# r9y9/deepvoice3_pytorch

Hardware: AMD Instinct MI355X
Metric: mel-frames/sec/node (train step, deepvoice3_ljspeech) (higher is better)
Workload: dtype f16x3

## Files before the change

### deepvoice3_pytorch_amd/csrc/api.hip

```cpp
#include "common.h"
#include <atomic>
#include <mutex>
#include <vector>
#include <string.h>

static thread_local char g_err[512] = "";

void dv3_set_error(const char* fmt, ...) {
  va_list ap;
  va_start(ap, fmt);
  vsnprintf(g_err, sizeof(g_err), fmt, ap);
  va_end(ap);
}

int g_dv3_last_conv = 0, g_dv3_last_wgrad = 0;

__device__ uint32_t g_dv3_range_events;
uint32_t* dv3_range_ctr() {
  static uint32_t* ptr = nullptr;
  static std::once_flag once;
  std::call_once(once, [] {
    void* p = nullptr;
    if (hipGetSymbolAddress(&p, HIP_SYMBOL(g_dv3_range_events)) == hipSuccess) ptr = (uint32_t*)p;
  });
// ... 194 lines not shown

extern "C" int dv3_device_info(int dev, char* name, int name_len, int* n_cu) {
  hipDeviceProp_t prop;
  hipError_t e = hipGetDeviceProperties(&prop, dev);
  if (e != hipSuccess) {
    dv3_set_error("hipGetDeviceProperties: %s", hipGetErrorString(e));
    return DV3_ELAUNCH;
  }
  if (name && name_len > 0) {
    strncpy(name, prop.gcnArchName, (size_t)name_len - 1);
    name[name_len - 1] = 0;
  }
  if (n_cu) *n_cu = prop.multiProcessorCount;
  return DV3_OK;
}

extern "C" int dv3_sizeof(const char* name) {
#define DV3_SZ(T) if (!strcmp(name, #T)) return (int)sizeof(T)
  DV3_SZ(dv3_conv_desc);
  DV3_SZ(dv3_wgrad_desc);
  DV3_SZ(dv3_wn_desc);
  DV3_SZ(dv3_wn_bwd_desc);
  DV3_SZ(dv3_gate_bwd_desc);
  DV3_SZ(dv3_softmax_desc);
  DV3_SZ(dv3_softmax_bwd_desc);
  DV3_SZ(dv3_spec_loss_desc);
  DV3_SZ(dv3_spec_items_desc);
  DV3_SZ(dv3_wn_multi_entry);
  DV3_SZ(dv3_conv_step_desc);
  DV3_SZ(dv3_attn_step_desc);
  DV3_SZ(dv3_decode_entry);
  DV3_SZ(dv3_decode_program);
  DV3_SZ(dv3_attn_fwd_desc);
  DV3_SZ(dv3_spk_layer);
  DV3_SZ(dv3_spk_desc);
  DV3_SZ(dv3_dropout_site);
  DV3_SZ(dv3_dtw_desc);
#undef DV3_SZ
  return -1;
}
```

### deepvoice3_pytorch_amd/csrc/attention.hip

```cpp
#include "common.h"

namespace {

__global__ __launch_bounds__(256) void attn_softmax_kernel(const dv3_softmax_desc p) {
  const int lane = threadIdx.x & 63;
  const int64_t row = (int64_t)blockIdx.x * 4 + (threadIdx.x >> 6);
  if (row >= (int64_t)p.B * p.Tq) return;
  const int b = (int)(row / p.Tq);
  const int Tk = p.Tk;
  float* s = p.s + row * Tk;
  int lo = 0, hi = Tk;
  if (p.key_len) hi = min(hi, p.key_len[b]);
  if (p.last_attended) {
    const int la = p.last_attended[0];
    const int wlo = la - p.win_back, whi = la + p.win_ahead;
    if (wlo > 0) lo = max(lo, wlo);
    if (whi < Tk) hi = min(hi, whi);
  }
  float mx = -INFINITY;
  for (int n = lo + lane; n < hi; n += 64) mx = fmaxf(mx, s[n]);
  mx = dv3_wave_max(mx);
  float sum = 0.f;
  for (int n = lo + lane; n < hi; n += 64) sum += expf(s[n] - mx);
  sum = dv3_wave_sum(sum);
// ... 15 lines not shown
__global__ __launch_bounds__(256) void attn_softmax_bwd_kernel(const dv3_softmax_bwd_desc p) {
  const int lane = threadIdx.x & 63;
  const int64_t row = (int64_t)blockIdx.x * 4 + (threadIdx.x >> 6);
  if (row >= (int64_t)p.B * p.Tq) return;
  const int Tk = p.Tk;
  const float* pr = p.p + row * Tk;
  const float* dpd = p.dpd ? p.dpd + row * Tk : nullptr;
  const float* dpx = p.dp_direct ? p.dp_direct + row * Tk : nullptr;
  float* ds = p.ds + row * Tk;
  const float drop_scale = p.scale_dev ? p.drop_scale * p.scale_dev[0] : p.drop_scale;
  float dot = 0.f;
  for (int n = lane; n < Tk; n += 64) {
    float d = 0.f;
    if (dpd) {
      d = dpd[n] * drop_scale;
      if (p.mask && !dv3_keep(p.mask, row, p.mask_rs, n)) d = 0.f;
    }
    if (dpx) d += dpx[n];
    dot += d * pr[n];
  }
  dot = dv3_wave_sum(dot);
  for (int n = lane; n < Tk; n += 64) {
    float d = 0.f;
    if (dpd) {
      d = dpd[n] * drop_scale;
      if (p.mask && !dv3_keep(p.mask, row, p.mask_rs, n)) d = 0.f;
    }
    if (dpx) d += dpx[n];
    ds[n] = pr[n] * (d - dot);
  }
}

typedef float f32x2v __attribute__((ext_vector_type(2)));
__global__ __launch_bounds__(256) void attn_fwd_kernel(const dv3_attn_fwd_desc p) {
  extern __shared__ float sc[];
  const int tid = threadIdx.x, lane = tid & 63, wave = tid >> 6;
  const int l31 = lane & 31, lhi = lane >> 5;
  const int b = blockIdx.y, t0 = blockIdx.x * 32;
  const int E = p.E, Tq = p.Tq, Tk = p.Tk;
  const int ld = Tk + 1;
  const int nkt = (Tk + 31) / 32;
  const float* __restrict__ qb = p.q + (int64_t)b * E * Tq;
  const float* __restrict__ kb = p.k + (int64_t)b * E * Tk;
  const int tq = min(t0 + l31, Tq - 1);
  for (int kt = wave; kt < nkt; kt += 4) {
    const int n = min(kt * 32 + l31, Tk - 1);
    f32x16 acc;
#pragma unroll
    for (int r = 0; r < 16; ++r) acc[r] = 0.f;
    auto fetch1 = [&](int e0, float (&a)[16], float (&bv)[16]) __attribute__((always_inline)) {
#pragma unroll
      for (int i = 0; i < 16; ++i) {
        const int e = e0 + 2 * i + lhi;
        const int ee = min(e, E - 1);
        const float av = qb[(int64_t)ee * Tq + tq];
        bv[i] = kb[(int64_t)ee * Tk + n];
        a[i] = e < E ? av : 0.f;
      }
    };
    float a0[16], b0[16], a1[16], b1[16];
    fetch1(0, a0, b0);
    for (int e0 = 0; e0 < E; e0 += 64) {
      if (e0 + 32 < E) fetch1(e0 + 32, a1, b1);
#pragma unroll
      for (int i = 0; i < 16; ++i) acc = __builtin_amdgcn_mfma_f32_32x32x2f32(a0[i], b0[i], acc, 0, 0, 0);
      if (e0 + 32 >= E) break;
      if (e0 + 64 < E) fetch1(e0 + 64, a0, b0);
// ... 8 lines not shown
  }
  __syncthreads();
  {
    const int row = tid >> 3, sub = tid & 7;
    const int t = t0 + row;
    int hi = Tk;
    if (p.key_len) hi = min(hi, p.key_len[b]);
    float* s = sc + row * ld;
    float mx = -INFINITY;
    for (int n = sub; n < hi; n += 8) mx = fmaxf(mx, s[n]);
#pragma unroll
    for (int off = 4; off > 0; off >>= 1) mx = fmaxf(mx, __shfl_xor(mx, off, 64));
    float sum = 0.f;
    for (int n = sub; n < hi; n += 8) sum += expf(s[n] - mx);
#pragma unroll
    for (int off = 4; off > 0; off >>= 1) sum += __shfl_xor(sum, off, 64);
    const float inv = 1.0f / sum;
    const float pd_scale = p.pd_scale_dev ? p.pd_scale * p.pd_scale_dev[0] : p.pd_scale;
    const int64_t grow = (int64_t)b * Tq + t;
    for (int n = sub; n < Tk; n += 8) {
      float v = 0.f;
      if (n < hi) v = expf(s[n] - mx) * inv;
      float d = v;
      if (p.mask && t < Tq) d = dv3_keep(p.mask, grow, p.mask_rs, n) ? v * p.drop_scale : 0.f;
      d *= pd_scale;
      s[n] = d;
      if (t < Tq) {
        p.P[grow * Tk + n] = v;
        p.pd[grow * Tk + n] = d;
      }
    }
  }
  __syncthreads();
  const float* __restrict__ vtb = p.vT + (int64_t)b * Tk * E;
  for (int et = wave; et * 32 < E; et += 4) {
    const int e = min(et * 32 + l31, E - 1);
    f32x16 acc;
#pragma unroll
    for (int r = 0; r < 16; ++r) acc[r] = 0.f;
    auto fetch3 = [&](int n0, float (&a)[16], float (&bv)[16]) __attribute__((always_inline)) {
#pragma unroll
      for (int i = 0; i < 16; ++i) {
        const int n = n0 + 2 * i + lhi;
        const int nn = min(n, Tk - 1);
        const float av = vtb[(int64_t)nn * E + e];
        bv[i] = sc[l31 * ld + nn];
        a[i] = n < Tk ? av : 0.f;
      }
    };
    float a0[16], b0[16], a1[16], b1[16];
    fetch3(0, a0, b0);
    for (int n0 = 0; n0 < Tk; n0 += 64) {
      if (n0 + 32 < Tk) fetch3(n0 + 32, a1, b1);
#pragma unroll
      for (int i = 0; i < 16; ++i) acc = __builtin_amdgcn_mfma_f32_32x32x2f32(a0[i], b0[i], acc, 0, 0, 0);
      if (n0 + 32 >= Tk) break;
      if (n0 + 64 < Tk) fetch3(n0 + 64, a0, b0);
#pragma unroll
      for (int i = 0; i < 16; ++i) acc = __builtin_amdgcn_mfma_f32_32x32x2f32(a1[i], b1[i], acc, 0, 0, 0);
    }
    const int t = t0 + l31;
    if (t < Tq) {
#pragma unroll
      for (int r = 0; r < 16; ++r) {
        const int ec = et * 32 + (r & 3) + 8 * (r >> 2) + 4 * lhi;
        if (ec < E) p.ctx[((int64_t)b * E + ec) * Tq + t] = acc[r];
      }
    }
  }
}

__global__ __launch_bounds__(64) void attn_argmax_kernel(const float* __restrict__ p, int Tk,
                                                         int32_t* __restrict__ out) {
  const int lane = threadIdx.x;
  float best = -INFINITY;
  int bi = 0x7fffffff;
  for (int n = lane; n < Tk; n += 64) {
    const float v = p[n];
    if (v > best) { best = v; bi = n; }
  }
#pragma unroll
  for (int off = 32; off > 0; off >>= 1) {
    const float ov = __shfl_xor(best, off, 64);
    const int oi = __shfl_xor(bi, off, 64);
    if (ov > best || (ov == best && oi < bi)) { best = ov; bi = oi; }
  }
  if (lane == 0) out[0] = bi;
}

}

extern "C" int dv3_attn_softmax_f32(const dv3_softmax_desc* d, void* stream) {
  DV3_REQUIRE(d && d->s && d->B > 0 && d->Tq > 0 && d->Tk > 0, "attn_softmax: bad args");
  if (d->mask) DV3_REQUIRE(d->pd && d->mask_rs * 32 >= d->Tk, "attn_softmax: mask needs pd and a wide enough row stride");
  const int64_t rows = (int64_t)d->B * d->Tq;
  hipLaunchKernelGGL(attn_softmax_kernel, dim3((unsigned)dv3_cdiv64(rows, 4)), dim3(256), 0,
                     (hipStream_t)stream, *d);
  return dv3_check_launch("attn_softmax_f32");
}

extern "C" int dv3_attn_softmax_bwd_f32(const dv3_softmax_bwd_desc* d, void* stream) {
  DV3_REQUIRE(d && d->p && d->ds && (d->dpd || d->dp_direct), "attn_softmax_bwd: bad args");
  DV3_REQUIRE(d->B > 0 && d->Tq > 0 && d->Tk > 0, "attn_softmax_bwd: bad dims");
  const int64_t rows = (int64_t)d->B * d->Tq;
  hipLaunchKernelGGL(attn_softmax_bwd_kernel, dim3((unsigned)dv3_cdiv64(rows, 4)), dim3(256), 0,
                     (hipStream_t)stream, *d);
  return dv3_check_launch("attn_softmax_bwd_f32");
}

extern "C" int dv3_attn_fwd_f32(const dv3_attn_fwd_desc* d, void* stream) {
  DV3_REQUIRE(d && d->q && d->k && d->vT && d->ctx && d->P && d->pd, "attn_fwd: null pointer");
  DV3_REQUIRE(d->B > 0 && d->E > 0 && d->Tq > 0 && d->Tk > 0 && d->B <= 65535, "attn_fwd: bad dims");
  if (d->mask) DV3_REQUIRE(d->mask_rs * 32 >= d->Tk, "attn_fwd: mask row stride too small");
  const size_t lds = (size_t)32 * (d->Tk + 1) * sizeof(float);
  DV3_REQUIRE(lds <= 64 * 1024, "attn_fwd: Tk = %d too long for the fused kernel (use the unfused path)", d->Tk);
  hipLaunchKernelGGL(attn_fwd_kernel, dim3(dv3_cdiv(d->Tq, 32), d->B), dim3(256), lds, (hipStream_t)stream, *d);
  return dv3_check_launch("attn_fwd");
}

extern "C" int dv3_attn_argmax_i32(const float* p_row, int32_t Tk, int32_t* out, void* stream) {
  DV3_REQUIRE(p_row && out && Tk > 0, "attn_argmax: bad args");
  hipLaunchKernelGGL(attn_argmax_kernel, dim3(1), dim3(64), 0, (hipStream_t)stream, p_row, Tk, out);
  return dv3_check_launch("attn_argmax_i32");
}
```

### deepvoice3_pytorch_amd/ops.py

```python
import contextlib
import ctypes
import functools
import math

import torch

from . import _lib
from ._lib import CONSTS, STRUCTS, _env_flag, _env_int, _env_str

EPI_LINEAR = CONSTS["DV3_EPI_LINEAR"]
EPI_RELU = CONSTS["DV3_EPI_RELU"]
EPI_SIGMOID = CONSTS["DV3_EPI_SIGMOID"]
EPI_GLU = CONSTS["DV3_EPI_GLU"]
EPI_HIGHWAY = CONSTS["DV3_EPI_HIGHWAY"]
EPI_DGRAD = CONSTS["DV3_EPI_DGRAD"]
EPI_SOFTSIGN = CONSTS["DV3_EPI_SOFTSIGN"]
STORE_BCT = CONSTS["DV3_STORE_BCT"]
STORE_INTERLEAVE2 = CONSTS["DV3_STORE_INTERLEAVE2"]

_conv_desc = STRUCTS["dv3_conv_desc"]
_wgrad_desc = STRUCTS["dv3_wgrad_desc"]
_wn_desc = STRUCTS["dv3_wn_desc"]
_wn_bwd_desc = STRUCTS["dv3_wn_bwd_desc"]
_gate_bwd_desc = STRUCTS["dv3_gate_bwd_desc"]
_softmax_desc = STRUCTS["dv3_softmax_desc"]
_softmax_bwd_desc = STRUCTS["dv3_softmax_bwd_desc"]
_attn_fwd_desc = STRUCTS["dv3_attn_fwd_desc"]
_spec_loss_desc = STRUCTS["dv3_spec_loss_desc"]
_spec_items_desc = STRUCTS["dv3_spec_items_desc"]


_GEMM_MODES = ("f16x3", "bf16x3", "f32", "bf16")
_gemm_mode = _env_str("DV3_GEMM", "f16x3")
if _gemm_mode not in _GEMM_MODES:
    raise RuntimeError("DV3_GEMM must be one of %s" % (_GEMM_MODES,))


def set_gemm_precision(mode):
    global _gemm_mode
    if mode not in _GEMM_MODES:
        raise ValueError("gemm precision must be one of %s" % (_GEMM_MODES,))
    prev, _gemm_mode = _gemm_mode, mode
    return prev


def gemm_precision():
    return _gemm_mode


_raw_stream = getattr(torch._C, "_cuda_getCurrentRawStream", None)
_cur_device = getattr(torch._C, "_cuda_getDevice", None)
import threading as _threading


class _StreamOverride(_threading.local):
    handle = None


_stream_override = _StreamOverride()

# ... 289 lines not shown
            pk.fwd_s._dv3_f16 = f16
            e = tab[n]
            e.d.v, e.d.g, e.d.scale = v.data_ptr(), _ptr(g), pk.scale.data_ptr()
            e.d.lda, e.d.a_half, e.d.ldb = pk.lda, pk.a_half, pk.ldb
            e.d.O, e.d.I, e.d.J, e.d.transposed, e.d.glu_cg = O, I, J, 0, glu_cg
            e.d.fwd_dtype = SPLIT_F16 if f16 else SPLIT_BF16
            e.fwd_split, e.bwd_split = pk.fwd_s.data_ptr(), pk.bwd_s.data_ptr()
            first_row.append(rows)
            first_block.append(blocks)
            rows += O
            blocks += ((O + 31) // 32) * ((I + 31) // 32)
            max_j = max(max_j, J)
            self.by_id[id(v)] = (pk, v.data_ptr(), glu_cg)
        raw = torch.frombuffer(bytearray(bytes(tab)), dtype=torch.uint8)
        self.table = raw.to(dev)
        self.first_row = torch.tensor(first_row, dtype=torch.int32, device=dev)
        self.first_block = torch.tensor(first_block, dtype=torch.int32, device=dev)
        self.n, self.rows, self.blocks, self.max_j = len(layers), rows, blocks, max_j
        self.keep = layers

    def run(self):
        _lib.call("dv3_weight_norm_split_pack_multi", self.table.data_ptr(), self.first_row.data_ptr(),
                  self.first_block.data_ptr(), self.n, self.rows, self.blocks, self.max_j, _stream())

    def lookup(self, v, glu_cg):
        hit = self.by_id.get(id(v))
        if hit is None or hit[1] != v.data_ptr() or hit[2] != glu_cg or self.mode != _gemm_mode:
            return None
        return hit[0]


prepacked = None
fused_attention = _env_flag("DV3_FUSED_ATTN", True)


bf16_storage = _env_flag("DV3_BF16_STORAGE", True)


def zero_(t):
    _lib.call("dv3_memset_b8", t.data_ptr(), 0, t.numel() * t.element_size(), _stream())
    return t


def storage_c8():
    return bf16_storage and _gemm_mode == "bf16"


def c8_groups(C):
    return _round_up(C, 32) // 8


def is_c8(t):
    return t is not None and t.dim() == 4 and t.dtype == torch.bfloat16 and t.shape[-1] == 8


def _c8_empty(B, C, T, device):
    shape = (B, c8_groups(C), T, 8)
    t = torch.empty(shape, dtype=torch.bfloat16, device=device)
    if C % 32:
        G, g0 = c8_groups(C), C // 8
        _lib.call("dv3_memset_rows_b8", t.data_ptr() + g0 * T * 16, 0, B, (G - g0) * T * 16, G * T * 16, _stream())
    t._dv3_C = C
    return t


def _c8_C(t, C=None):
# ... 1207 lines not shown
    if (x8 or want8) and not _c8_layer_ok(v, cfg, x8 if want8 is None else bool(want8), x.shape[2]):
        y = ConvLayerFn.apply(from_c8(x, v.shape[1]) if x8 else x, v, g, bias, spk,
                              from_c8(r) if is_c8(r) else r, from_c8(r2) if is_c8(r2) else r2, cfg, packed)
        out8 = x8 if want8 is None else bool(want8)
        return to_c8(y) if out8 else y
    if x8 or want8:
        y = ConvLayerC8Fn.apply(x, v, g, bias, spk, r, r2, cfg, packed)
        if is_c8(y):
            gated = cfg.mode in (EPI_GLU, EPI_HIGHWAY)
            y._dv3_C = v.shape[0] // 2 if gated else v.shape[0]
        return y
    return ConvLayerFn.apply(x, v, g, bias, spk, r, r2, cfg, packed)


def _attn_split(forward=False):
    if forward and _gemm_mode == "f16x3":
        return False
    return _gemm_mode != "f32"


class AttnCoreFn(torch.autograd.Function):
    @staticmethod
    def forward(ctx, q, k, v, key_len, last_attended, cfg):
        q, k, v = _c(_chk(q, "q")), _c(_chk(k, "k")), _c(_chk(v, "v"))
        B, E, Tq = q.shape
        Tk = k.shape[2]
        p_drop, training, win_back, win_ahead, site = cfg
        dev = q.device
        bits, bits_rs, dscale = None, 0, 1.0
        if training and p_drop > 0:
            bits, bits_rs = dropout_bits(B * Tq, Tk, p_drop, dev, site)
            dscale = 1.0 / (1.0 - p_drop)
        if fused_attention and last_attended is None and Tk <= 511 and Tq > 1:
            vT = transpose(v)
            ctxv = torch.empty((B, E, Tq), dtype=torch.float32, device=dev)
            P = torch.empty((B, Tq, Tk), dtype=torch.float32, device=dev)
            pd = torch.empty_like(P)
            d = _attn_fwd_desc()
            d.q, d.k, d.vT, d.key_len = q.data_ptr(), k.data_ptr(), vT.data_ptr(), _ptr(key_len)
            d.mask, d.mask_rs, d.drop_scale = _ptr(bits), bits_rs, dscale
            vs = valid.scale if valid is not None else None
            d.pd_scale = 1.0 if vs is not None else Tk * math.sqrt(1.0 / Tk)
            d.pd_scale_dev = _ptr(vs)
            d.ctx, d.P, d.pd = ctxv.data_ptr(), P.data_ptr(), pd.data_ptr()
            d.B, d.E, d.Tq, d.Tk = B, E, Tq, Tk
            _lib.call("dv3_attn_fwd_f32", ctypes.byref(d), _stream())
            if any(ctx.needs_input_grad[:3]):
                ctx.save_for_backward(q, k, v, P, pd)
                ctx.bits, ctx.bits_rs, ctx.dscale, ctx.pd_scale = bits, bits_rs, dscale, d.pd_scale
                ctx.scale_dev = vs
            return ctxv, P
        S = conv_gemm(k, q, Tq, 0, B=B, Cin=E, Tin=Tk, M=Tq, Tout=Tk, a_bs=E * Tq)
        pd = torch.empty_like(S)
        d = _softmax_desc()
        d.s, d.pd, d.key_len, d.last_attended = S.data_ptr(), pd.data_ptr(), _ptr(key_len), _ptr(last_attended)
        d.mask, d.mask_rs, d.drop_scale = _ptr(bits), bits_rs, dscale
        vs = valid.scale if valid is not None else None
        d.pd_scale = 1.0 if vs is not None else Tk * math.sqrt(1.0 / Tk)
        d.pd_scale_dev = _ptr(vs)
        d.B, d.Tq, d.Tk, d.win_back, d.win_ahead = B, Tq, Tk, win_back, win_ahead
        _lib.call("dv3_attn_softmax_f32", ctypes.byref(d), _stream())
        P = S
        ctxv = wgrad_gemm(v, pd, B=B, M=E, Cin=Tq, T=Tk, Tin=Tk, n_slabs=B,
                          split_bf16=_attn_split(forward=True)).view(B, E, Tq)
        if any(ctx.needs_input_grad[:3]):
            ctx.save_for_backward(q, k, v, P, pd)
            ctx.bits, ctx.bits_rs, ctx.dscale, ctx.pd_scale = bits, bits_rs, dscale, d.pd_scale
            ctx.scale_dev = vs
        return ctxv, P

    @staticmethod
    def backward(ctx, dctx, dP):
        q, k, v, P, pd = ctx.saved_tensors
        B, E, Tq = q.shape
        Tk = k.shape[2]
        dctx = _c(dctx)
        pdT = transpose(pd)
        dv = wgrad_gemm(dctx, pdT, B=B, M=E, Cin=Tk, T=Tq, Tin=Tq, n_slabs=B, split_bf16=_attn_split()).view(B, E, Tk)
        dpd = conv_gemm(v, dctx, Tq, 0, B=B, Cin=E, Tin=Tk, M=Tq, Tout=Tk, a_bs=E * Tq)
        dS = torch.empty_like(P)
        d = _softmax_bwd_desc()
        d.p, d.dpd, d.ds = P.data_ptr(), dpd.data_ptr(), dS.data_ptr()
        d.dp_direct = _ptr(_c(dP)) if dP is not None else None
        d.mask, d.mask_rs, d.drop_scale = _ptr(ctx.bits), ctx.bits_rs, ctx.dscale * ctx.pd_scale
        d.scale_dev = _ptr(ctx.scale_dev)
        d.B, d.Tq, d.Tk = B, Tq, Tk
        _lib.call("dv3_attn_softmax_bwd_f32", ctypes.byref(d), _stream())
        dq = wgrad_gemm(k, dS, B=B, M=E, Cin=Tq, T=Tk, Tin=Tk, n_slabs=B, split_bf16=_attn_split()).view(B, E, Tq)
        dST = transpose(dS)
        dk = wgrad_gemm(q, dST, B=B, M=E, Cin=Tk, T=Tq, Tin=Tq, n_slabs=B, split_bf16=_attn_split()).view(B, E, Tk)
        return dq, dk, dv, None, None, None


def attention_core(q, k, v, key_len=None, last_attended=None, p=0.0, training=False, win_back=1,
                   win_ahead=3, site=None):
    return AttnCoreFn.apply(q, k, v, key_len, last_attended, (p, training, win_back, win_ahead, site))


class EmbeddingBCTFn(torch.autograd.Function):
    @staticmethod
    def forward(ctx, idx, weight, p, training, padding_idx, site):
        _chk(weight, "embedding weight")
        idx = _c(idx.long())
        B, T = idx.shape
        n_vocab, C = weight.shape
        out = torch.empty((B, C, T), dtype=torch.float32, device=weight.device)
        bits, rs, dscale = None, 0, 1.0
        if training and p > 0:
            bits, rs = dropout_bits(B * C, T, p, weight.device, site)
# ... 639 lines not shown
```

### include/dv3hip.h

```cpp
#ifndef DV3HIP_H
#define DV3HIP_H

#include <stdint.h>

#ifdef __cplusplus
extern "C" {
#endif

#define DV3_OK 0
#define DV3_EINVAL (-1)
#define DV3_ELAUNCH (-2)

#define DV3_ABI_VERSION 49
int dv3_abi_version(void);
const char* dv3_last_error(void);
int dv3_device_info(int dev, char* name, int name_len, int* n_cu);
int dv3_sizeof(const char* name);
int dv3_debug_set(int what, int value);
int dv3_debug_read(int what, void* dst, int64_t bytes);
int dv3_debug_get(int what);

int dv3_ring_standin(const void* src, int64_t src_bytes, void* scratch, int64_t scratch_bytes, int64_t bytes,
                     int32_t channels, int32_t threads, float bytes_per_us, void* stream);

// ... 174 lines not shown
int dv3_dropout_keep_c8_multi(const dv3_dropout_site* sites, int32_t n, uint64_t seed,
                              const uint64_t* dev_seed_offset, void* stream);

int dv3_dropout_apply_f32(const float* x, const uint32_t* bits, int32_t bits_rs, float scale,
                          float* out, int64_t rows, int32_t T, void* stream);

typedef struct dv3_softmax_desc {
  float* s; float* pd;
  const int32_t* key_len;
  const int32_t* last_attended;
  const uint32_t* mask; int32_t mask_rs; float drop_scale;
  float pd_scale;
  int32_t B, Tq, Tk, win_back, win_ahead;
  const float* pd_scale_dev;
} dv3_softmax_desc;
int dv3_attn_softmax_f32(const dv3_softmax_desc* d, void* stream);
typedef struct dv3_softmax_bwd_desc {
  const float* p; const float* dpd; const float* dp_direct; float* ds;
  const uint32_t* mask; int32_t mask_rs; float drop_scale;
  int32_t B, Tq, Tk;
  const float* scale_dev;
} dv3_softmax_bwd_desc;
int dv3_attn_softmax_bwd_f32(const dv3_softmax_bwd_desc* d, void* stream);
typedef struct dv3_attn_fwd_desc {
  const float* q; const float* k; const float* vT;
  const int32_t* key_len;
  const uint32_t* mask; int32_t mask_rs; float drop_scale;
  float pd_scale;
  float* ctx; float* P; float* pd;
  int32_t B, E, Tq, Tk;
  const float* pd_scale_dev;
} dv3_attn_fwd_desc;
int dv3_attn_fwd_f32(const dv3_attn_fwd_desc* d, void* stream);
int dv3_attn_argmax_i32(const float* p_row, int32_t Tk, int32_t* out, void* stream);

int dv3_transpose_f32(const float* x, float* y, const float* add, int32_t B, int32_t R,
                      int32_t C, float alpha, void* stream);
int dv3_axpby_f32(const float* a, const float* b, float* out, int64_t n, float alpha,
                  void* stream);
int dv3_sum_scalars_f32(const float* a, const float* b, const float* c, const float* d, float* out, void* stream);
int dv3_memset_b8(void* p, int32_t value, int64_t bytes, void* stream);
int dv3_memset_rows_b8(void* p, int32_t value, int64_t rows, int64_t row_bytes, int64_t row_stride_bytes, void* stream);
int dv3_zero_tail_b32(void* x, int64_t rows, int32_t T, int32_t words, const int32_t* t_valid, int32_t mult,
                      int32_t max_tail, void* stream);
int dv3_zero_tail_items_b32(void* x, int32_t B, int64_t rows_per_item, int32_t T, int32_t words, const int32_t* len,
                            int32_t mult, int32_t max_tail, void* stream);
int dv3_embedding_bct_f32(const int64_t* idx, const float* w, float* out,
                          const uint32_t* mask, int32_t mask_rs, float drop_scale,
                          int32_t B, int32_t T, int32_t C, int32_t n_vocab, void* stream);
int dv3_embedding_bct_bwd_f32(const int64_t* idx, const float* dout, float* dw,
                              const uint32_t* mask, int32_t mask_rs, float drop_scale,
                              int32_t B, int32_t T, int32_t C, int32_t n_vocab,
                              int32_t padding_idx, void* stream);
int dv3_sincos_pos_bct_f32(const int64_t* pos, const float* table, const float* w,
                           int32_t w_per_batch, const float* base, float* out, int32_t B,
                           int32_t T, int32_t C, int32_t n_pos, int32_t apply_sincos,
                           void* stream);
int dv3_sincos_pos_table_bwd_f32(const int64_t* pos, const float* table, const float* w, int32_t w_per_batch,
                                 const float* dout, float* dtable, int32_t B, int32_t T, int32_t C,
                                 int32_t n_pos, int32_t apply_sincos, void* stream);
int dv3_sincos_pos_bwd_f32(const int64_t* pos, const float* table, const float* w,
                           int32_t w_per_batch, const float* dout, float* dw, int32_t B, int32_t T,
                           int32_t C, int32_t n_pos, void* stream);
int dv3_sincos_pos_bwd2_f32(const int64_t* pos, const float* table, const float* w,
                            int32_t w_per_batch, const float* dout, float* partial, int32_t n_chunks, float* dw,
                            int32_t B, int32_t T, int32_t C, int32_t n_pos, void* stream);
// ... 239 lines not shown
```

Measured before the change: 3.782 million.

## Fuse attention backward into two kernels and read V without transpose in forward

Adds a fused attention backward made of two kernels. The first computes dP = dctx·V, the softmax backward and dq in one kernel per query tile. The second computes dv and dk with a split-bf16 MFMA GEMM. This replaces the former chain of transposes, wgrad/conv GEMMs and a separate softmax-backward launch, and is meant to cut launches, intermediate buffers and transposes at the cost of a large amount of new code. The forward now reads V in (B,E,Tk) layout with vector loads, which removes the explicit transpose.

```diff
diff --git a/deepvoice3_pytorch_amd/csrc/api.hip b/deepvoice3_pytorch_amd/csrc/api.hip
--- a/deepvoice3_pytorch_amd/csrc/api.hip
+++ b/deepvoice3_pytorch_amd/csrc/api.hip
@@ -250,6 +250,7 @@
   DV3_SZ(dv3_decode_entry);
   DV3_SZ(dv3_decode_program);
   DV3_SZ(dv3_attn_fwd_desc);
+  DV3_SZ(dv3_attn_bwd_desc);
   DV3_SZ(dv3_spk_layer);
   DV3_SZ(dv3_spk_desc);
   DV3_SZ(dv3_dropout_site);
diff --git a/deepvoice3_pytorch_amd/csrc/attention.hip b/deepvoice3_pytorch_amd/csrc/attention.hip
--- a/deepvoice3_pytorch_amd/csrc/attention.hip
+++ b/deepvoice3_pytorch_amd/csrc/attention.hip
@@ -71,7 +71,9 @@
 }
 
 typedef float f32x2v __attribute__((ext_vector_type(2)));
-__global__ __launch_bounds__(256) void attn_fwd_kernel(const dv3_attn_fwd_desc p) {
+typedef float f32x4uv __attribute__((ext_vector_type(4), aligned(4)));
+template <bool VB>
+__global__ __launch_bounds__(256) void attn_fwd_kernel(const dv3_attn_fwd_desc p, const float* __restrict__ v_bct) {
   extern __shared__ float sc[];
   const int tid = threadIdx.x, lane = tid & 63, wave = tid >> 6;
   const int l31 = lane & 31, lhi = lane >> 5;
@@ -146,18 +148,30 @@
     }
   }
   __syncthreads();
-  const float* __restrict__ vtb = p.vT + (int64_t)b * Tk * E;
+  const float* __restrict__ vtb = VB ? v_bct + (int64_t)b * E * Tk : p.vT + (int64_t)b * Tk * E;
   for (int et = wave; et * 32 < E; et += 4) {
     const int e = min(et * 32 + l31, E - 1);
     f32x16 acc;
 #pragma unroll
     for (int r = 0; r < 16; ++r) acc[r] = 0.f;
     auto fetch3 = [&](int n0, float (&a)[16], float (&bv)[16]) __attribute__((always_inline)) {
+      if (VB && n0 + 32 <= Tk) {
+        const float* __restrict__ vr = vtb + (int64_t)e * Tk + n0;
+        f32x4uv x[8];
+#pragma unroll
+        for (int j = 0; j < 8; ++j) x[j] = *reinterpret_cast<const f32x4uv*>(vr + 4 * j);
+#pragma unroll
+        for (int i = 0; i < 16; ++i) {
+          a[i] = lhi ? x[i >> 1][2 * (i & 1) + 1] : x[i >> 1][2 * (i & 1)];
+          bv[i] = sc[l31 * ld + n0 + 2 * i + lhi];
+        }
+        return;
+      }
 #pragma unroll
       for (int i = 0; i < 16; ++i) {
         const int n = n0 + 2 * i + lhi;
         const int nn = min(n, Tk - 1);
-        const float av = vtb[(int64_t)nn * E + e];
+        const float av = VB ? vtb[(int64_t)e * Tk + nn] : vtb[(int64_t)nn * E + e];
         bv[i] = sc[l31 * ld + nn];
         a[i] = n < Tk ? av : 0.f;
       }
@@ -222,14 +236,27 @@
   return dv3_check_launch("attn_softmax_bwd_f32");
 }
 
-extern "C" int dv3_attn_fwd_f32(const dv3_attn_fwd_desc* d, void* stream) {
-  DV3_REQUIRE(d && d->q && d->k && d->vT && d->ctx && d->P && d->pd, "attn_fwd: null pointer");
+static int attn_fwd_launch(const dv3_attn_fwd_desc* d, const float* v_bct, void* stream) {
+  DV3_REQUIRE(d && d->q && d->k && d->ctx && d->P && d->pd, "attn_fwd: null pointer");
+  DV3_REQUIRE((d->vT != nullptr) != (v_bct != nullptr), "attn_fwd: exactly one of vT (B,Tk,E) and v (B,E,Tk)");
   DV3_REQUIRE(d->B > 0 && d->E > 0 && d->Tq > 0 && d->Tk > 0 && d->B <= 65535, "attn_fwd: bad dims");
   if (d->mask) DV3_REQUIRE(d->mask_rs * 32 >= d->Tk, "attn_fwd: mask row stride too small");
   const size_t lds = (size_t)32 * (d->Tk + 1) * sizeof(float);
   DV3_REQUIRE(lds <= 64 * 1024, "attn_fwd: Tk = %d too long for the fused kernel (use the unfused path)", d->Tk);
-  hipLaunchKernelGGL(attn_fwd_kernel, dim3(dv3_cdiv(d->Tq, 32), d->B), dim3(256), lds, (hipStream_t)stream, *d);
+  const dim3 grid(dv3_cdiv(d->Tq, 32), d->B);
+  if (v_bct) {
+    hipLaunchKernelGGL(attn_fwd_kernel<true>, grid, dim3(256), lds, (hipStream_t)stream, *d, v_bct);
+  } else {
+    hipLaunchKernelGGL(attn_fwd_kernel<false>, grid, dim3(256), lds, (hipStream_t)stream, *d, v_bct);
+  }
   return dv3_check_launch("attn_fwd");
+}
+
+extern "C" int dv3_attn_fwd_f32(const dv3_attn_fwd_desc* d, void* stream) { return attn_fwd_launch(d, nullptr, stream); }
+
+extern "C" int dv3_attn_fwd_bct_f32(const dv3_attn_fwd_desc* d, const float* v, void* stream) {
+  DV3_REQUIRE(v, "attn_fwd_bct: null v");
+  return attn_fwd_launch(d, v, stream);
 }
 
 extern "C" int dv3_attn_argmax_i32(const float* p_row, int32_t Tk, int32_t* out, void* stream) {
diff --git a/deepvoice3_pytorch_amd/csrc/attention_bwd.hip b/deepvoice3_pytorch_amd/csrc/attention_bwd.hip
--- /dev/null
+++ b/deepvoice3_pytorch_amd/csrc/attention_bwd.hip
@@ -0,0 +1,505 @@
+#include "common.h"
+#include <type_traits>
+
+typedef __bf16 bf16x8 __attribute__((ext_vector_type(8)));
+typedef __bf16 bf16x2 __attribute__((ext_vector_type(2)));
+typedef float f32x2 __attribute__((ext_vector_type(2)));
+typedef float f32x4u __attribute__((ext_vector_type(4), aligned(4)));
+
+namespace {
+
+__device__ __forceinline__ void split8(const float (&v)[8], bf16x8& hi, bf16x8& lo) {
+#pragma unroll
+  for (int i = 0; i < 8; i += 2) {
+    const f32x2 f = {v[i], v[i + 1]};
+    const bf16x2 h = __builtin_convertvector(f, bf16x2);
+    const f32x2 r = f - __builtin_convertvector(h, f32x2);
+    const bf16x2 l = __builtin_convertvector(r, bf16x2);
+    hi[i] = h[0]; hi[i + 1] = h[1];
+    lo[i] = l[0]; lo[i + 1] = l[1];
+  }
+}
+
+__device__ __forceinline__ void load8_row(const float* __restrict__ row, int n, int len, float (&v)[8]) {
+  if (n + 8 <= len) {
+    const f32x4u a = *reinterpret_cast<const f32x4u*>(row + n);
+    const f32x4u b = *reinterpret_cast<const f32x4u*>(row + n + 4);
+    v[0] = a[0]; v[1] = a[1]; v[2] = a[2]; v[3] = a[3];
+    v[4] = b[0]; v[5] = b[1]; v[6] = b[2]; v[7] = b[3];
+  } else {
+#pragma unroll
+    for (int e = 0; e < 8; ++e) {
+      const float x = row[min(n + e, len - 1)];
+      v[e] = n + e < len ? x : 0.f;
+    }
+  }
+}
+
+__device__ __host__ __forceinline__ bool attn_bwd_small(int M, int Cin) { return M <= 64 && Cin <= 64; }
+
+template <int TERMS>
+__device__ __forceinline__ void mfma_terms(f32x16& acc, bf16x8 ah, bf16x8 al, bf16x8 bh, bf16x8 bl) {
+  if (TERMS == 3) {
+    acc = __builtin_amdgcn_mfma_f32_32x32x16_bf16(al, bh, acc, 0, 0, 0);
+    acc = __builtin_amdgcn_mfma_f32_32x32x16_bf16(ah, bl, acc, 0, 0, 0);
+  }
+  acc = __builtin_amdgcn_mfma_f32_32x32x16_bf16(ah, bh, acc, 0, 0, 0);
+}
+
+template <int TERMS>
+__global__ __launch_bounds__(256) void attn_bwd_q_kernel(const dv3_attn_bwd_desc p) {
+  extern __shared__ __attribute__((aligned(16))) float sc[];
+  const int tid = threadIdx.x, lane = tid & 63, wave = tid >> 6;
+  const int l31 = lane & 31, lhi = lane >> 5;
+  const int b = blockIdx.y, t0 = blockIdx.x * 32;
+  const int E = p.E, Tq = p.Tq, Tk = p.Tk;
+  const int ld = Tk + 1;
+  const int nkt = (Tk + 31) / 32;
+  const float* __restrict__ gb = p.dctx + (int64_t)b * E * Tq;
+  const float* __restrict__ vb = p.v + (int64_t)b * E * Tk;
+  const int tq = min(t0 + l31, Tq - 1);
+  for (int kt = wave; kt < nkt; kt += 4) {
+    const int n = min(kt * 32 + l31, Tk - 1);
+    f32x16 acc;
+#pragma unroll
+    for (int r = 0; r < 16; ++r) acc[r] = 0.f;
+    auto fetch1 = [&](int e0, float (&a)[16], float (&bv)[16]) __attribute__((always_inline)) {
+#pragma unroll
+      for (int i = 0; i < 16; ++i) {
+        const int e = e0 + 2 * i + lhi;
+        const int ee = min(e, E - 1);
+        const float av = gb[(int64_t)ee * Tq + tq];
+        const float xv = vb[(int64_t)ee * Tk + n];
+        a[i] = e < E ? av : 0.f;
+        bv[i] = e < E ? xv : 0.f;
+      }
+    };
+    float a0[16], b0[16], a1[16], b1[16];
+    fetch1(0, a0, b0);
+    for (int e0 = 0; e0 < E; e0 += 64) {
+      if (e0 + 32 < E) fetch1(e0 + 32, a1, b1);
+#pragma unroll
+      for (int i = 0; i < 16; ++i) acc = __builtin_amdgcn_mfma_f32_32x32x2f32(a0[i], b0[i], acc, 0, 0, 0);
+      if (e0 + 32 >= E) break;
+      if (e0 + 64 < E) fetch1(e0 + 64, a0, b0);
+#pragma unroll
+      for (int i = 0; i < 16; ++i) acc = __builtin_amdgcn_mfma_f32_32x32x2f32(a1[i], b1[i], acc, 0, 0, 0);
+    }
+    const int col = kt * 32 + l31;
+    if (col < Tk) {
+#pragma unroll
+      for (int r = 0; r < 16; ++r) sc[((r & 3) + 8 * (r >> 2) + 4 * lhi) * ld + col] = acc[r];
+    }
+  }
+  __syncthreads();
+  {
+    constexpr int MC = 8;
+    const int nc = (Tk + 63) >> 6;
+    const float drop_scale = p.scale_dev ? p.drop_scale * p.scale_dev[0] : p.drop_scale;
+    float pv[2][MC], xv[2][MC];
+    uint32_t kv[2][MC];
+    auto fetch = [&](int rr, float (&pw)[MC], float (&xw)[MC], uint32_t (&kw)[MC]) __attribute__((always_inline)) {
+      const int64_t row = (int64_t)b * Tq + min(t0 + rr, Tq - 1);
+#pragma unroll
+      for (int c = 0; c < MC; ++c) {
+        if (c < nc) {
+          const int nn = min(lane + 64 * c, Tk - 1);
+          pw[c] = p.P[row * Tk + nn];
+          xw[c] = p.dP ? p.dP[row * Tk + nn] : 0.f;
+          kw[c] = p.mask ? p.mask[row * p.mask_rs + (nn >> 5)] : 0xffffffffu;
+        }
+      }
+    };
+    auto reduce_row = [&](int rr, const float (&pw)[MC], const float (&xw)[MC], const uint32_t (&kw)[MC])
+        __attribute__((always_inline)) {
+      float* s = sc + rr * ld;
+      const int t = t0 + rr;
+      if (t >= Tq) {
+        for (int n = lane; n < Tk; n += 64) s[n] = 0.f;
+        return;
+      }
+      float* ds = p.dS + ((int64_t)b * Tq + t) * Tk;
+      float dd[MC];
+      float dot = 0.f;
+#pragma unroll
+      for (int c = 0; c < MC; ++c) {
+        const int n = lane + 64 * c;
+        if (c < nc && n < Tk) {
+          float d = s[n] * drop_scale;
+          if (p.mask && !((kw[c] >> (n & 31)) & 1u)) d = 0.f;
+          if (p.dP) d += xw[c];
+          dot += d * pw[c];
+          dd[c] = d;
+        }
+      }
+      dot = dv3_wave_sum(dot);
+#pragma unroll
+      for (int c = 0; c < MC; ++c) {
+        const int n = lane + 64 * c;
+        if (c < nc && n < Tk) {
+          const float o = pw[c] * (dd[c] - dot);
+          ds[n] = o;
+          s[n] = o;
+        }
+      }
+    };
+    fetch(wave, pv[0], xv[0], kv[0]);
+#pragma unroll
+    for (int i = 0; i < 8; i += 2) {
+      fetch(wave + 4 * (i + 1), pv[1], xv[1], kv[1]);
+      reduce_row(wave + 4 * i, pv[0], xv[0], kv[0]);
+      if (i + 2 < 8) fetch(wave + 4 * (i + 2), pv[0], xv[0], kv[0]);
+      reduce_row(wave + 4 * (i + 1), pv[1], xv[1], kv[1]);
+    }
+  }
+  __syncthreads();
+  const float* __restrict__ kb = p.k + (int64_t)b * E * Tk;
+  if (attn_bwd_small(E, Tq)) {
+    for (int et = wave; et * 32 < E; et += 4) {
+      const float* __restrict__ krow = kb + (int64_t)min(et * 32 + l31, E - 1) * Tk;
+      f32x16 acc;
+#pragma unroll
+      for (int r = 0; r < 16; ++r) acc[r] = 0.f;
+      for (int n0 = 0; n0 < Tk; n0 += 2) {
+        const int n = n0 + lhi, nn = min(n, Tk - 1);
+        const float av = krow[nn], xv = sc[l31 * ld + nn];
+        acc = __builtin_amdgcn_mfma_f32_32x32x2f32(n < Tk ? av : 0.f, n < Tk ? xv : 0.f, acc, 0, 0, 0);
+      }
+      const int t = t0 + l31;
+      if (t < Tq) {
+#pragma unroll
+        for (int r = 0; r < 16; ++r) {
+          const int ec = et * 32 + (r & 3) + 8 * (r >> 2) + 4 * lhi;
+          if (ec < E) p.dq[((int64_t)b * E + ec) * Tq + t] = acc[r];
+        }
+      }
+    }
+    return;
+  }
+  const int nk8 = nkt * 4;
+  bf16x8* img = reinterpret_cast<bf16x8*>(sc);
+  {
+    constexpr int MAXU = 8;
+    bf16x8 uh[MAXU], ul[MAXU];
+#pragma unroll
+    for (int i = 0; i < MAXU; ++i) {
+      const int u = tid + i * 256;
+      if (u < nk8 * 32) {
+        const int k8 = u >> 5, rr = u & 31;
+        float x[8];
+#pragma unroll
+        for (int e = 0; e < 8; ++e) {
+          const int n = k8 * 8 + e;
+          const float y = sc[rr * ld + min(n, Tk - 1)];
+          x[e] = n < Tk ? y : 0.f;
+        }
+        split8(x, uh[i], ul[i]);
+      }
+    }
+    __syncthreads();
+#pragma unroll
+    for (int i = 0; i < MAXU; ++i) {
+      const int u = tid + i * 256;
+      if (u < nk8 * 32) {
+        img[u] = uh[i];
+        if (TERMS == 3) img[nk8 * 32 + u] = ul[i];
+      }
+    }
+  }
+  __syncthreads();
+  for (int et0 = 2 * wave; et0 * 32 < E; et0 += 8) {
+    const float* __restrict__ krow[2];
+#pragma unroll
+    for (int h = 0; h < 2; ++h) krow[h] = kb + (int64_t)min((et0 + h) * 32 + l31, E - 1) * Tk;
+    f32x16 acc[2];
+#pragma unroll
+    for (int h = 0; h < 2; ++h)
+#pragma unroll
+      for (int r = 0; r < 16; ++r) acc[h][r] = 0.f;
+    float ra[2][2][8], rn[2][2][8];
+#pragma unroll
+    for (int h = 0; h < 2; ++h)
+#pragma unroll
+      for (int ks = 0; ks < 2; ++ks) load8_row(krow[h], 16 * ks + 8 * lhi, Tk, ra[h][ks]);
+    for (int kbk = 0; kbk < nkt; ++kbk) {
+      if (kbk + 1 < nkt) {
+#pragma unroll
+        for (int h = 0; h < 2; ++h)
+#pragma unroll
+          for (int ks = 0; ks < 2; ++ks) load8_row(krow[h], (kbk + 1) * 32 + 16 * ks + 8 * lhi, Tk, rn[h][ks]);
+      }
+#pragma unroll
+      for (int ks = 0; ks < 2; ++ks) {
+        const int bi = (kbk * 4 + 2 * ks + lhi) * 32 + l31;
+        const bf16x8 bh = img[bi];
+        bf16x8 bl = bh;
+        if (TERMS == 3) bl = img[nk8 * 32 + bi];
+#pragma unroll
+        for (int h = 0; h < 2; ++h) {
+          bf16x8 ah, al;
+          split8(ra[h][ks], ah, al);
+          mfma_terms<TERMS>(acc[h], ah, al, bh, bl);
+        }
+      }
+      if (kbk + 1 < nkt) {
+#pragma unroll
+        for (int h = 0; h < 2; ++h)
+#pragma unroll
+          for (int ks = 0; ks < 2; ++ks)
+#pragma unroll
+            for (int e = 0; e < 8; ++e) ra[h][ks][e] = rn[h][ks][e];
+      }
+    }
+    const int t = t0 + l31;
+    if (t < Tq) {
+#pragma unroll
+      for (int h = 0; h < 2; ++h)
+#pragma unroll
+        for (int r = 0; r < 16; ++r) {
+          const int ec = (et0 + h) * 32 + (r & 3) + 8 * (r >> 2) + 4 * lhi;
+          if (ec < E) p.dq[((int64_t)b * E + ec) * Tq + t] = acc[h][r];
+        }
+    }
+  }
+}
+
+__device__ __forceinline__ uint32_t valid8(int t, int len) {
+  const int elo = max(0, -t), ehi = min(8, len - t);
+  return ehi > elo ? (((1u << ehi) - 1u) & ~((1u << elo) - 1u)) : 0u;
+}
+__device__ __forceinline__ void mask8(float (&v)[8], uint32_t m) {
+#pragma unroll
+  for (int e = 0; e < 8; ++e)
+    v[e] = __uint_as_float(__float_as_uint(v[e]) & (uint32_t)__builtin_amdgcn_sbfe((int)m, e, 1));
+}
+__device__ __forceinline__ void load8_raw(const float* __restrict__ base, int off, int total, float (&v)[8]) {
+  const bool inside = off <= total - 8;
+  if (__all(inside)) {
+    const f32x4u a = *reinterpret_cast<const f32x4u*>(base + off);
+    const f32x4u b = *reinterpret_cast<const f32x4u*>(base + off + 4);
+    v[0] = a[0]; v[1] = a[1]; v[2] = a[2]; v[3] = a[3];
+    v[4] = b[0]; v[5] = b[1]; v[6] = b[2]; v[7] = b[3];
+  } else {
+#pragma unroll
+    for (int e = 0; e < 8; ++e) v[e] = base[min(off + e, total - 1)];
+  }
+}
+
+template <int TERMS>
+__global__ __launch_bounds__(256, 2) void attn_bwd_kv_kernel(const dv3_attn_bwd_desc p) {
+  constexpr int BM = 128, BN = 128, NT = 256, KB = 4, PAD = 2, BKT = 32;
+  constexpr int LDM = BM + PAD, LDN = BN + PAD;
+  constexpr int BUF = 2 * KB * LDM + 2 * KB * LDN;
+  __shared__ __attribute__((aligned(16))) bf16x8 smem[2 * BUF];
+  const int tid = threadIdx.x, lane = tid & 63;
+  const int wave = __builtin_amdgcn_readfirstlane(tid >> 6);
+  const int wm = wave >> 1, wn = wave & 1;
+  const int l31 = lane & 31, lhi = lane >> 5;
+  const int E = p.E, Tq = p.Tq, Tk = p.Tk;
+  const int m_tiles = (E + BM - 1) / BM, n_tiles = (Tk + BN - 1) / BN;
+  int pid = blockIdx.x;
+  const int mt = pid % m_tiles; pid /= m_tiles;
+  const int nt = pid % n_tiles;
+  const int prod = pid / n_tiles;
+  const int b = blockIdx.y;
+  const int m0 = mt * BM, c0 = nt * BN;
+  const float* __restrict__ G = (prod ? p.q : p.dctx) + (int64_t)b * E * Tq;
+  const float* __restrict__ X = (prod ? p.dS : p.pd) + (int64_t)b * Tq * Tk;
+  float* __restrict__ O = (prod ? p.dk : p.dv) + (int64_t)b * E * Tk;
+
+  if (attn_bwd_small(E, Tk)) {
+    const int et = wave >> 1, n0 = (wave & 1) * 32;
+    if (et * 32 >= E || n0 >= Tk) return;
+    const int nc = min(n0 + l31, Tk - 1);
+    const bool n_ok = n0 + l31 < Tk;
+    const int64_t eo = (int64_t)min(et * 32 + l31, E - 1) * Tq;
+    f32x16 acc;
+#pragma unroll
+    for (int r = 0; r < 16; ++r) acc[r] = 0.f;
+    for (int t0 = 0; t0 < Tq; t0 += 2) {
+      const int t = t0 + lhi, tt = min(t, Tq - 1);
+      const bool ok = t < Tq;
+      const float g = G[eo + tt];
+      const float x = X[(int64_t)tt * Tk + nc];
+      acc = __builtin_amdgcn_mfma_f32_32x32x2f32(ok ? g : 0.f, (ok && n_ok) ? x : 0.f, acc, 0, 0, 0);
+    }
+    if (n_ok) {
+#pragma unroll
+      for (int r = 0; r < 16; ++r) {
+        const int ec = et * 32 + (r & 3) + 8 * (r >> 2) + 4 * lhi;
+        if (ec < E) O[(int64_t)ec * Tk + n0 + l31] = acc[r];
+      }
+    }
+    return;
+  }
+
+  constexpr int GU = BM * KB / NT, XU = BN * KB / NT;
+  int grow[GU], gk8[GU], xrow[XU], xk8[XU];
+  int grow_off[GU], xcol[XU];
+  bool grow_ok[GU], xrow_ok[XU];
+#pragma unroll
+  for (int u = 0; u < GU; ++u) {
+    const int idx = tid + u * NT;
+    grow[u] = idx >> 2;
+    gk8[u] = idx & 3;
+    const int m = m0 + grow[u];
+    grow_ok[u] = m < E;
+    grow_off[u] = (m < E ? m : E - 1) * Tq + gk8[u] * 8;
+  }
+#pragma unroll
+  for (int u = 0; u < XU; ++u) {
+    const int idx = tid + u * NT;
+    xrow[u] = idx & (BN - 1);
+    xk8[u] = idx >> 7;
+    const int c = c0 + xrow[u];
+    xrow_ok[u] = c < Tk;
+    xcol[u] = c < Tk ? c : Tk - 1;
+  }
+  const int g_total = E * Tq;
+  const int nsteps = (Tq + BKT - 1) / BKT;
+  float rg[2][GU][8], rx[2][XU][8];
+
+  auto load_step = [&](int step, auto set_c) {
+    constexpr int S = decltype(set_c)::value;
+    const int t0 = step * BKT;
+#pragma unroll
+    for (int u = 0; u < GU; ++u) load8_raw(G, grow_off[u] + t0, g_total, rg[S][u]);
+#pragma unroll
+    for (int u = 0; u < XU; ++u) {
+#pragma unroll
+      for (int e = 0; e < 8; ++e) rx[S][u][e] = X[min(t0 + xk8[u] * 8 + e, Tq - 1) * Tk + xcol[u]];
+    }
+  };
+  auto write_step = [&](int step, int buf, auto set_c) {
+    constexpr int S = decltype(set_c)::value;
+    const int t0 = step * BKT;
+    const bool edge = t0 + BKT > Tq;
+    bf16x8* dst = smem + buf * BUF;
+#pragma unroll
+    for (int u = 0; u < GU; ++u) {
+      uint32_t vm = 0xffu;
+      if (edge) vm = valid8(t0 + gk8[u] * 8, Tq);
+      if (!grow_ok[u]) vm = 0u;
+      if (__any(vm != 0xffu)) mask8(rg[S][u], vm);
+      bf16x8 hi, lo;
+      split8(rg[S][u], hi, lo);
+      const int o = gk8[u] * LDM + grow[u];
+      dst[o] = hi;
+      if (TERMS == 3) dst[KB * LDM + o] = lo;
+    }
+    bf16x8* dx = dst + 2 * KB * LDM;
+#pragma unroll
+    for (int u = 0; u < XU; ++u) {
+      uint32_t vm = 0xffu;
+      if (edge) vm = valid8(t0 + xk8[u] * 8, Tq);
+      if (!xrow_ok[u]) vm = 0u;
+      if (__any(vm != 0xffu)) mask8(rx[S][u], vm);
+      bf16x8 hi, lo;
+      split8(rx[S][u], hi, lo);
+      const int o = xk8[u] * LDN + xrow[u];
+      dx[o] = hi;
+      if (TERMS == 3) dx[KB * LDN + o] = lo;
+    }
+  };
+
+  f32x16 acc[2][2];
+#pragma unroll
+  for (int a = 0; a < 2; ++a)
+#pragma unroll
+    for (int bq = 0; bq < 2; ++bq)
+#pragma unroll
+      for (int r = 0; r < 16; ++r) acc[a][bq][r] = 0.f;
+
+  auto mfma_step = [&](int cur) {
+    const bf16x8* GsH = smem + cur * BUF;
+    const bf16x8* GsL = GsH + KB * LDM;
+    const bf16x8* XsH = GsH + 2 * KB * LDM;
+    const bf16x8* XsL = XsH + KB * LDN;
+#pragma unroll
+    for (int ks = 0; ks < 2; ++ks) {
+      const int k8 = 2 * ks + lhi;
+      const int ai = k8 * LDM + wm * 64 + l31;
+      const int xi = k8 * LDN + wn * 64 + l31;
+      const bf16x8 ah0 = GsH[ai], ah1 = GsH[ai + 32];
+      const bf16x8 bh0 = XsH[xi], bh1 = XsH[xi + 32];
+      if (TERMS == 1) {
+        acc[0][0] = __builtin_amdgcn_mfma_f32_32x32x16_bf16(ah0, bh0, acc[0][0], 0, 0, 0);
+        acc[0][1] = __builtin_amdgcn_mfma_f32_32x32x16_bf16(ah0, bh1, acc[0][1], 0, 0, 0);
+        acc[1][0] = __builtin_amdgcn_mfma_f32_32x32x16_bf16(ah1, bh0, acc[1][0], 0, 0, 0);
+        acc[1][1] = __builtin_amdgcn_mfma_f32_32x32x16_bf16(ah1, bh1, acc[1][1], 0, 0, 0);
+        continue;
+      }
+      const bf16x8 al0 = GsL[ai], al1 = GsL[ai + 32];
+      const bf16x8 bl0 = XsL[xi], bl1 = XsL[xi + 32];
+      acc[0][0] = __builtin_amdgcn_mfma_f32_32x32x16_bf16(al0, bh0, acc[0][0], 0, 0, 0);
+      acc[0][1] = __builtin_amdgcn_mfma_f32_32x32x16_bf16(al0, bh1, acc[0][1], 0, 0, 0);
+      acc[1][0] = __builtin_amdgcn_mfma_f32_32x32x16_bf16(al1, bh0, acc[1][0], 0, 0, 0);
+      acc[1][1] = __builtin_amdgcn_mfma_f32_32x32x16_bf16(al1, bh1, acc[1][1], 0, 0, 0);
+      acc[0][0] = __builtin_amdgcn_mfma_f32_32x32x16_bf16(ah0, bl0, acc[0][0], 0, 0, 0);
+      acc[0][1] = __builtin_amdgcn_mfma_f32_32x32x16_bf16(ah0, bl1, acc[0][1], 0, 0, 0);
+      acc[1][0] = __builtin_amdgcn_mfma_f32_32x32x16_bf16(ah1, bl0, acc[1][0], 0, 0, 0);
+      acc[1][1] = __builtin_amdgcn_mfma_f32_32x32x16_bf16(ah1, bl1, acc[1][1], 0, 0, 0);
+      acc[0][0] = __builtin_amdgcn_mfma_f32_32x32x16_bf16(ah0, bh0, acc[0][0], 0, 0, 0);
+      acc[0][1] = __builtin_amdgcn_mfma_f32_32x32x16_bf16(ah0, bh1, acc[0][1], 0, 0, 0);
+      acc[1][0] = __builtin_amdgcn_mfma_f32_32x32x16_bf16(ah1, bh0, acc[1][0], 0, 0, 0);
+      acc[1][1] = __builtin_amdgcn_mfma_f32_32x32x16_bf16(ah1, bh1, acc[1][1], 0, 0, 0);
+    }
+  };
+  using S0 = std::integral_constant<int, 0>;
+  using S1 = std::integral_constant<int, 1>;
+
+  load_step(0, S0{});
+  write_step(0, 0, S0{});
+  if (nsteps > 1) load_step(1, S1{});
+  __syncthreads();
+  for (int step = 0; step < nsteps; step += 2) {
+    if (step + 2 < nsteps) load_step(step + 2, S0{});
+    mfma_step(0);
+    if (step + 1 < nsteps) write_step(step + 1, 1, S1{});
+    __syncthreads();
+    if (step + 1 >= nsteps) break;
+    if (step + 3 < nsteps) load_step(step + 3, S1{});
+    mfma_step(1);
+    if (step + 2 < nsteps) write_step(step + 2, 0, S0{});
+    __syncthreads();
+  }
+#pragma unroll
+  for (int mi = 0; mi < 2; ++mi)
+#pragma unroll
+    for (int ni = 0; ni < 2; ++ni) {
+      const int c = c0 + wn * 64 + ni * 32 + l31;
+      if (c >= Tk) continue;
+#pragma unroll
+      for (int r = 0; r < 16; ++r) {
+        const int m = m0 + wm * 64 + mi * 32 + (r & 3) + 8 * (r >> 2) + 4 * lhi;
+        if (m < E) O[(int64_t)m * Tk + c] = acc[mi][ni][r];
+      }
+    }
+}
+
+}
+
+extern "C" int dv3_attn_bwd_f32(const dv3_attn_bwd_desc* d, void* stream) {
+  DV3_REQUIRE(d && d->q && d->k && d->v && d->dctx && d->P && d->pd && d->dq && d->dk && d->dv && d->dS,
+              "attn_bwd: null pointer");
+  DV3_REQUIRE(d->B > 0 && d->E > 0 && d->Tq > 1 && d->Tk > 0 && d->B <= 65535, "attn_bwd: bad dims");
+  DV3_REQUIRE((int64_t)d->B * d->E * (d->Tq > d->Tk ? d->Tq : d->Tk) < (1ll << 30) &&
+                  (int64_t)d->B * d->Tq * d->Tk < (1ll << 30),
+              "attn_bwd: a tensor of 2^30 elements or more (use the unfused path)");
+  DV3_REQUIRE(d->Tk <= 511, "attn_bwd: Tk = %d too long for the fused kernels (use the unfused path)", d->Tk);
+  DV3_REQUIRE(d->terms == 3 || d->terms == 1, "attn_bwd: terms must be 3 (split bf16) or 1 (bf16)");
+  if (d->mask) DV3_REQUIRE(d->mask_rs * 32 >= d->Tk, "attn_bwd: mask row stride too small");
+  hipStream_t st = (hipStream_t)stream;
+  const size_t tile = (size_t)32 * (d->Tk + 1) * sizeof(float);
+  const size_t image = (size_t)(d->terms == 3 ? 2 : 1) * dv3_cdiv(d->Tk, 32) * 4 * 32 * 16;
+  const size_t lds = tile > image ? tile : image;
+  const dim3 ga(dv3_cdiv(d->Tq, 32), d->B), gb(dv3_cdiv(d->E, 128) * dv3_cdiv(d->Tk, 128) * 2, d->B);
+  if (d->terms == 3) {
+    hipLaunchKernelGGL(attn_bwd_q_kernel<3>, ga, dim3(256), lds, st, *d);
+    hipLaunchKernelGGL(attn_bwd_kv_kernel<3>, gb, dim3(256), 0, st, *d);
+  } else {
+    hipLaunchKernelGGL(attn_bwd_q_kernel<1>, ga, dim3(256), lds, st, *d);
+    hipLaunchKernelGGL(attn_bwd_kv_kernel<1>, gb, dim3(256), 0, st, *d);
+  }
+  return dv3_check_launch("attn_bwd");
+}
diff --git a/deepvoice3_pytorch_amd/ops.py b/deepvoice3_pytorch_amd/ops.py
--- a/deepvoice3_pytorch_amd/ops.py
+++ b/deepvoice3_pytorch_amd/ops.py
@@ -26,6 +26,7 @@
 _softmax_desc = STRUCTS["dv3_softmax_desc"]
 _softmax_bwd_desc = STRUCTS["dv3_softmax_bwd_desc"]
 _attn_fwd_desc = STRUCTS["dv3_attn_fwd_desc"]
+_attn_bwd_desc = STRUCTS["dv3_attn_bwd_desc"]
 _spec_loss_desc = STRUCTS["dv3_spec_loss_desc"]
 _spec_items_desc = STRUCTS["dv3_spec_items_desc"]
 
@@ -381,6 +382,7 @@
 
 prepacked = None
 fused_attention = _env_flag("DV3_FUSED_ATTN", True)
+fused_attention_bwd = _env_flag("DV3_FUSED_ATTN_BWD", True)
 
 
 bf16_storage = _env_flag("DV3_BF16_STORAGE", True)
@@ -1654,19 +1656,18 @@
             bits, bits_rs = dropout_bits(B * Tq, Tk, p_drop, dev, site)
             dscale = 1.0 / (1.0 - p_drop)
         if fused_attention and last_attended is None and Tk <= 511 and Tq > 1:
-            vT = transpose(v)
             ctxv = torch.empty((B, E, Tq), dtype=torch.float32, device=dev)
             P = torch.empty((B, Tq, Tk), dtype=torch.float32, device=dev)
             pd = torch.empty_like(P)
             d = _attn_fwd_desc()
-            d.q, d.k, d.vT, d.key_len = q.data_ptr(), k.data_ptr(), vT.data_ptr(), _ptr(key_len)
+            d.q, d.k, d.vT, d.key_len = q.data_ptr(), k.data_ptr(), None, _ptr(key_len)
             d.mask, d.mask_rs, d.drop_scale = _ptr(bits), bits_rs, dscale
             vs = valid.scale if valid is not None else None
             d.pd_scale = 1.0 if vs is not None else Tk * math.sqrt(1.0 / Tk)
             d.pd_scale_dev = _ptr(vs)
             d.ctx, d.P, d.pd = ctxv.data_ptr(), P.data_ptr(), pd.data_ptr()
             d.B, d.E, d.Tq, d.Tk = B, E, Tq, Tk
-            _lib.call("dv3_attn_fwd_f32", ctypes.byref(d), _stream())
+            _lib.call("dv3_attn_fwd_bct_f32", ctypes.byref(d), v.data_ptr(), _stream())
             if any(ctx.needs_input_grad[:3]):
                 ctx.save_for_backward(q, k, v, P, pd)
                 ctx.bits, ctx.bits_rs, ctx.dscale, ctx.pd_scale = bits, bits_rs, dscale, d.pd_scale
@@ -1697,6 +1698,19 @@
         B, E, Tq = q.shape
         Tk = k.shape[2]
         dctx = _c(dctx)
+        if (fused_attention_bwd and _attn_split() and Tk <= 511 and Tq > 1
+                and max(q.numel(), k.numel(), P.numel()) < 2 ** 30):
+            dq, dk, dv, dS = torch.empty_like(q), torch.empty_like(k), torch.empty_like(v), torch.empty_like(P)
+            d = _attn_bwd_desc()
+            d.q, d.k, d.v, d.dctx = q.data_ptr(), k.data_ptr(), v.data_ptr(), dctx.data_ptr()
+            d.P, d.pd, d.dP = P.data_ptr(), pd.data_ptr(), (_ptr(_c(dP)) if dP is not None else None)
+            d.mask, d.mask_rs, d.drop_scale = _ptr(ctx.bits), ctx.bits_rs, ctx.dscale * ctx.pd_scale
+            d.scale_dev = _ptr(ctx.scale_dev)
+            d.dq, d.dk, d.dv, d.dS = dq.data_ptr(), dk.data_ptr(), dv.data_ptr(), dS.data_ptr()
+            d.B, d.E, d.Tq, d.Tk = B, E, Tq, Tk
+            d.terms = 1 if _gemm_mode == "bf16" else 3
+            _lib.call("dv3_attn_bwd_f32", ctypes.byref(d), _stream())
+            return dq, dk, dv, None, None, None
         pdT = transpose(pd)
         dv = wgrad_gemm(dctx, pdT, B=B, M=E, Cin=Tk, T=Tq, Tin=Tq, n_slabs=B, split_bf16=_attn_split()).view(B, E, Tk)
         dpd = conv_gemm(v, dctx, Tq, 0, B=B, Cin=E, Tin=Tk, M=Tq, Tout=Tk, a_bs=E * Tq)
diff --git a/include/dv3hip.h b/include/dv3hip.h
--- a/include/dv3hip.h
+++ b/include/dv3hip.h
@@ -230,6 +230,17 @@
   const float* pd_scale_dev;
 } dv3_attn_fwd_desc;
 int dv3_attn_fwd_f32(const dv3_attn_fwd_desc* d, void* stream);
+int dv3_attn_fwd_bct_f32(const dv3_attn_fwd_desc* d, const float* v, void* stream);
+typedef struct dv3_attn_bwd_desc {
+  const float* q; const float* k; const float* v;
+  const float* dctx; const float* P; const float* pd; const float* dP;
+  const uint32_t* mask; int32_t mask_rs; float drop_scale;
+  const float* scale_dev;
+  float* dq; float* dk; float* dv; float* dS;
+  int32_t B, E, Tq, Tk;
+  int32_t terms;
+} dv3_attn_bwd_desc;
+int dv3_attn_bwd_f32(const dv3_attn_bwd_desc* d, void* stream);
 int dv3_attn_argmax_i32(const float* p_row, int32_t Tk, int32_t* out, void* stream);
 
 int dv3_transpose_f32(const float* x, float* y, const float* add, int32_t B, int32_t R,
```

New measurement: 3.804 million, median of 6. No clear change (+0.6%).
